# lixirui142/VidToMe

Hardware: AMD Instinct MI355X
Metric: denoising steps/sec, 16-frame 512x512 SD-1.5 chunk, ratio=0.5 (higher is better)
Workload: dtype f16 tokens; matching f16-MFMA filter + f32 exact refine (f32-identical indices); attention f16 MFMA with f32 accumulate

## Files before the change

vidtome_amd/csrc/match_filter.hip:

```cpp
#include "common.h"
#include "ablate.h"
#include "match_plan.h"

#include <algorithm>
#include <type_traits>

namespace {

using namespace vtm_match_plan;
static_assert(MODE_SCOUT_RANGE == VTM_MATCH_SCOUT_RANGE, "match_plan.h restates the public mode value");
constexpr int THREADS = 256;
constexpr float SCALE = 1024.0f;
constexpr float INV_S2 = 1.0f / (1024.0f * 1024.0f);
constexpr float WINDOW = SRC_LO ? 6.5e-4f : DST_LO ? 1.5e-3f : 2.4e-3f;
constexpr int MAX_C = 1280;

typedef float f32x16 __attribute__((ext_vector_type(16)));
typedef _Float16 h16x8 __attribute__((ext_vector_type(8)));
typedef uint32_t u32x4 __attribute__((ext_vector_type(4)));
typedef __attribute__((address_space(3))) void lds_void;
typedef const __attribute__((address_space(1))) void glb_void;

using vtm::to_f32;

template <typename T>
__device__ __forceinline__ const T *pool_row(const T *x0, int64_t P0, const T *x1, int64_t P1, int64_t b,
                                             int64_t r, int64_t C) {
    return r < P0 ? x0 + (b * P0 + r) * C : x1 + (b * P1 + (r - P0)) * C;
}

template <typename T>
__device__ __forceinline__ void load8(const T *src, float (&f)[8]) {
    if constexpr (sizeof(T) == 4) {
        const float4 v0 = *reinterpret_cast<const float4 *>(src);
        const float4 v1 = *reinterpret_cast<const float4 *>(src + 4);
        f[0] = v0.x; f[1] = v0.y; f[2] = v0.z; f[3] = v0.w;
        f[4] = v1.x; f[5] = v1.y; f[6] = v1.z; f[7] = v1.w;
    } else {
        const uint4 v = *reinterpret_cast<const uint4 *>(src);
        const T *e = reinterpret_cast<const T *>(&v);
#pragma unroll
        for (int j = 0; j < 8; ++j) f[j] = to_f32(e[j]);
    }
}

__device__ __forceinline__ float vmax3(float a, float b, float c) {
    float d;
    asm("v_max3_f32 %0, %1, %2, %3" : "=v"(d) : "v"(a), "v"(b), "v"(c));
    return d;
}
__device__ __forceinline__ float vmax2(float a, float b) {
    float d;
    asm("v_max_f32 %0, %1, %2" : "=v"(d) : "v"(a), "v"(b));
    return d;
}

struct RowDivisor {
    float n, r1, lo;
};
__device__ __forceinline__ RowDivisor row_divisor(float n) {
    const float r = __builtin_amdgcn_rcpf(n);
    const float e = __builtin_fmaf(-n, r, 1.0f);
    return {n, __builtin_fmaf(e, r, r), fmaxf(0x1p-102f, n * 0x1p-124f)};
}
__device__ __forceinline__ bool div_ok(float x, const RowDivisor &d) { return __builtin_fabsf(x) >= d.lo || x == 0.0f; }
__device__ __forceinline__ float div_by_row(float x, const RowDivisor &d) {
    const float q = x * d.r1;
    const float t = __builtin_fmaf(-d.n, q, x);
    const float q1 = __builtin_fmaf(t, d.r1, q);
    const float t2 = __builtin_fmaf(-d.n, q1, x);
    return __builtin_fmaf(t2, d.r1, q1);
}

__device__ __forceinline__ uint32_t orderable(float f) {
    if (f != f) return 0xffffffffu;
    const uint32_t u = __float_as_uint(f + 0.0f);
    return (u & 0x80000000u) ? ~u : (u | 0x80000000u);
}
__device__ __forceinline__ float from_orderable(uint32_t o) {
    if (o == 0u) return -INFINITY;
    return __uint_as_float((o & 0x80000000u) ? (o & 0x7fffffffu) : ~o);
}

struct SplitArgs {
    const int32_t *rows;
    int64_t n;
    float *norms;
    uint4 *out_hi, *out_lo;
    int64_t n_pad;
    float *rest, *tile_rest;
    float *rest2, *tile_rest2;
};

#ifndef VTM_PREP_PIECES
#define VTM_PREP_PIECES 10
#endif
constexpr int PREP_PIECES = VTM_PREP_PIECES;
constexpr int PREP_STRIDE = PREP_PIECES * 16 + 16;

template <typename T>
__global__ __launch_bounds__(64 * PREP_WAVES) void prep_operand(const T *__restrict__ x0, int64_t P0,
                                                    const T *__restrict__ x1, int64_t P1, int64_t B, int64_t C,
                                                    SplitArgs A0, SplitArgs A1, int64_t C_pad,
                                                    uint32_t *__restrict__ zero, int64_t zero_words,
                                                    unsigned long long *__restrict__ best, int64_t nbest, int64_t cut,
                                                    int64_t cut2) {
    static_assert(sizeof(T) == 2 || sizeof(T) == 4, "element size");
    static_assert(PREP_WAVES % 2 == 0, "a 128-row tile is two waves of one workgroup");
    __shared__ float wave_rest[PREP_WAVES], wave_rest2[PREP_WAVES];
    constexpr int EPP = 16 / (int)sizeof(T);
    __shared__ __attribute__((aligned(16))) char slab[PREP_WAVES][64 * PREP_STRIDE];
    const int64_t G = C_pad / 8;
    const int64_t gid = (int64_t)blockIdx.x * blockDim.x + threadIdx.x, gsz = (int64_t)gridDim.x * blockDim.x;
    for (int64_t w = gid; w < zero_words; w += gsz) zero[w] = 0u;
    for (int64_t w = gid; w < nbest; w += gsz) best[w] = 0ull;
    const int lane = threadIdx.x & 63, wave = threadIdx.x >> 6;
    char *my = slab[wave];

    int64_t idx = gid;
    const bool second = idx >= B * A0.n_pad;
    if (second) idx -= B * A0.n_pad;
    const SplitArgs &A = second ? A1 : A0;
    const int64_t n = A.n, n_pad = A.n_pad;
    const bool in_range = idx < B * n_pad;
    const int64_t i = in_range ? idx % n_pad : 0, b = in_range ? idx / n_pad : 0;
    const bool real = in_range && i < n;
    const T *src = real ? pool_row(x0, P0, x1, P1, b, A.rows[b * n + i], C) : x0;

    const int pieces = (int)(C * sizeof(T) / 16);
    const int nchunks = (pieces + PREP_PIECES - 1) / PREP_PIECES;
    uint4 stage[PREP_PIECES];
    auto issue = [&](int chunk) {
#pragma unroll
        for (int t = 0; t < PREP_PIECES; ++t) {
            const int q = lane + 64 * t, r = q / PREP_PIECES, col = q % PREP_PIECES;
            const T *rp = reinterpret_cast<const T *>(__shfl((unsigned long long)reinterpret_cast<uintptr_t>(src), r, 64));
            const int piece = chunk * PREP_PIECES + col;
            stage[t] = piece < pieces ? *reinterpret_cast<const uint4 *>(rp + (int64_t)piece * EPP) : make_uint4(0, 0, 0, 0);
        }
    };
    auto to_lds = [&]() {
#pragma unroll
        for (int t = 0; t < PREP_PIECES; ++t) {
            const int q = lane + 64 * t, r = q / PREP_PIECES, col = q % PREP_PIECES;
            *reinterpret_cast<uint4 *>(my + r * PREP_STRIDE + col * 16) = stage[t];
        }
    };
    auto my_piece = [&](int col, float (&f)[EPP]) {
        const uint4 v = *reinterpret_cast<const uint4 *>(my + lane * PREP_STRIDE + col * 16);
        const T *e = reinterpret_cast<const T *>(&v);
#pragma unroll
        for (int k = 0; k < EPP; ++k) f[k] = to_f32(e[k]);
    };

    float acc = 0.0f;
    issue(0);
    for (int c = 0; c < nchunks; ++c) {
        to_lds();
        if (c + 1 < nchunks) issue(c + 1);
        const int valid = min(PREP_PIECES, pieces - c * PREP_PIECES);
        for (int col = 0; col < valid; ++col) {
            float f[EPP];
            my_piece(col, f);
#pragma unroll
            for (int k = 0; k < EPP; ++k) acc = __builtin_fmaf(f[k], f[k], acc);
        }
    }
    const float nrm = __builtin_sqrtf(acc);
    if (real) A.norms[b * n + i] = nrm;

    const float rscale = SCALE * __builtin_amdgcn_rcpf(nrm);
    uint4 *__restrict__ out_hi = in_range ? A.out_hi + (b * G) * n_pad + i : nullptr;
    uint4 *__restrict__ out_lo = (in_range && A.out_lo) ? A.out_lo + (b * G) * n_pad + i : nullptr;
    constexpr int PPG = 8 / EPP;
    float rest = 0.0f, rest2 = 0.0f;
    issue(0);
    for (int c = 0; c < nchunks; ++c) {
        to_lds();
        if (c + 1 < nchunks) issue(c + 1);
        const int valid = min(PREP_PIECES, pieces - c * PREP_PIECES);
        for (int col = 0; col + PPG <= valid; col += PPG) {
            float f[8];
            if constexpr (PPG == 1) {
                my_piece(col, f);
            } else {
                float f0[EPP], f1[EPP];
                my_piece(col, f0);
                my_piece(col + 1, f1);
#pragma unroll
                for (int k = 0; k < EPP; ++k) { f[k] = f0[k]; f[EPP + k] = f1[k]; }
            }
            uint4 vh, vl;
            _Float16 *ph = reinterpret_cast<_Float16 *>(&vh), *pl = reinterpret_cast<_Float16 *>(&vl);
#pragma unroll
            for (int e = 0; e < 8; ++e) {
                const float sc = DST_LO ? (f[e] / nrm) * SCALE : f[e] * rscale;
                const _Float16 h = (_Float16)sc;
                ph[e] = h;
                pl[e] = (_Float16)(sc - (float)h);
            }
            if (!real) vh = vl = make_uint4(0, 0, 0, 0);
            const int64_t g = ((int64_t)c * PREP_PIECES + col) / PPG;
            if (g * 8 >= cut2) {
                float sq = 0.0f;
#pragma unroll
                for (int e = 0; e < 8; ++e) sq = __builtin_fmaf((float)ph[e], (float)ph[e], sq);
                rest2 += sq;
                if (g * 8 >= cut) rest += sq;
            }
            if (in_range) {
                out_hi[g * n_pad] = vh;
                if (out_lo) out_lo[g * n_pad] = vl;
            }
        }
    }
    if (in_range)
        for (int64_t g = C / 8; g < G; ++g) {
            out_hi[g * n_pad] = make_uint4(0, 0, 0, 0);
            if (out_lo) out_lo[g * n_pad] = make_uint4(0, 0, 0, 0);
        }
    const bool bad_row = real && !(nrm >= 0x1p-100f && nrm <= 0x1p100f);
    const float rnorm = !real ? 0.0f : bad_row ? INFINITY : __builtin_sqrtf(rest) * (1.0f + 0x1p-16f);
    if (in_range && A.rest) A.rest[b * n_pad + i] = rnorm;
    float wm = rnorm;
#pragma unroll
    for (int off = 32; off > 0; off >>= 1) wm = fmaxf(wm, __shfl_xor(wm, off, 64));
    if (lane == 0) wave_rest[wave] = wm;
    const float rnorm2 = !real ? 0.0f : bad_row ? INFINITY : __builtin_sqrtf(rest2) * (1.0f + 0x1p-16f);
    if (in_range && A.rest2) A.rest2[b * n_pad + i] = rnorm2;
    float wm2 = rnorm2;
#pragma unroll
    for (int off = 32; off > 0; off >>= 1) wm2 = fmaxf(wm2, __shfl_xor(wm2, off, 64));
    if (lane == 0) wave_rest2[wave] = wm2;
    __syncthreads();
    if (in_range && A.tile_rest && (threadIdx.x & 127) == 0)
        A.tile_rest[(b * n_pad + i) / 128] = fmaxf(wave_rest[wave], wave_rest[wave + 1]);
    if (in_range && A.tile_rest2 && (threadIdx.x & 127) == 0)
        A.tile_rest2[(b * n_pad + i) / 128] = fmaxf(wave_rest2[wave], wave_rest2[wave + 1]);
}

template <bool SCOUT>
__global__ __launch_bounds__(THREADS, 2) void filter_kernel(
    const uint4 *__restrict__ ah, const uint4 *__restrict__ al, const uint4 *__restrict__ bh,
    const uint4 *__restrict__ bl, int64_t Ns, int64_t Nd, int64_t Ns_pad, int64_t Nd_pad, int64_t C_pad, int align,
    int ns_tiles, int nd_tiles, int nsplit, int tiles_per_split, int total_src_tiles, int patch_tiles,
    unsigned int *__restrict__ amax, int *__restrict__ cnt, uint2 *__restrict__ cand, int cand_rows, int *__restrict__ flags,
    const float *__restrict__ rest_a, const float *__restrict__ rest_bt, int KP, int count_blocks,
    unsigned int *__restrict__ tilemap, int map_words) {
    __shared__ __attribute__((aligned(16))) uint4 sA[2][DST_LO ? 2 : 1][8 * FBD];

    const int tid = threadIdx.x, lane = tid & 63;
    const int wave = __builtin_amdgcn_readfirstlane(tid >> 6);
    const int l31 = lane & 31, kh = lane >> 5;

    const int xcd = blockIdx.x & 7, slot = blockIdx.x >> 3;
    const int per_group = patch_tiles * nsplit;
    const int grp = (slot / per_group) * 8 + xcd;
    const int q = slot % per_group;
    const int stg = grp * patch_tiles + q % patch_tiles;
    const int split = q / patch_tiles;
    if (stg >= total_src_tiles) return;
    const int st_ = stg % ns_tiles;
    const int bi = stg / ns_tiles;
    int jt0 = split * tiles_per_split;
    int jt1 = min(jt0 + tiles_per_split, nd_tiles);
    if (jt0 >= jt1) return;
    if constexpr (!SCOUT) {
        if (tilemap != nullptr) {
            const unsigned int *row = tilemap + (int64_t)stg * map_words;
            int lo = jt1, hi = jt0;
            for (int w = jt0 >> 5; w <= (jt1 - 1) >> 5; ++w) {
                unsigned int bits = row[w];
                if (w == (jt0 >> 5)) bits &= 0xffffffffu << (jt0 & 31);
                if (w == ((jt1 - 1) >> 5) && (jt1 & 31)) bits &= 0xffffffffu >> (32 - (jt1 & 31));
                if (bits) {
                    lo = min(lo, w * 32 + __ffs(bits) - 1);
                    hi = max(hi, w * 32 + 32 - __clz(bits));
                }
            }
            lo = __builtin_amdgcn_readfirstlane(lo);
            hi = __builtin_amdgcn_readfirstlane(hi);
            if (lo >= hi) return;
            jt0 = lo;
            jt1 = hi;
        }
    }

    const int KT = SCOUT ? KP : (int)(C_pad / FBK);
    const int64_t G = C_pad / 8;
    const int steps = (jt1 - jt0) * KT;
    int n_tested = 0, n_alive = 0;
    const uint4 *srch = ah + (int64_t)bi * G * Ns_pad, *srcl = al + (int64_t)bi * G * Ns_pad;
    const uint4 *dsth = bh + (int64_t)bi * G * Nd_pad, *dstl = bl + (int64_t)bi * G * Nd_pad;
    const int64_t srow0 = (int64_t)st_ * FBS + wave * 64;

    constexpr int NB = SRC_LO ? 4 : 2;
    const uint32_t voff_b = (uint32_t)(kh * Ns_pad + srow0 + l31) * 16u;
    const int64_t bgroup = 2 * Ns_pad;
    u32x4 rb[4][2][2];
    [[maybe_unused]] auto load_b = [&](int kt, int ks, u32x4 (&dst)[2][2]) {
        const uint4 *ph = srch + (int64_t)ABL_STREAMED(kt * 4 + ks, ks) * bgroup;
        asm volatile("global_load_dwordx4 %0, %1, %2" : "=v"(dst[0][0]) : "v"(voff_b), "s"(ph));
        asm volatile("global_load_dwordx4 %0, %1, %2 offset:512" : "=v"(dst[1][0]) : "v"(voff_b), "s"(ph));
        if constexpr (SRC_LO) {
            const uint4 *pl = srcl + (int64_t)(kt * 4 + ks) * bgroup;
            asm volatile("global_load_dwordx4 %0, %1, %2" : "=v"(dst[0][1]) : "v"(voff_b), "s"(pl));
            asm volatile("global_load_dwordx4 %0, %1, %2 offset:512" : "=v"(dst[1][1]) : "v"(voff_b), "s"(pl));
        }
    };
    auto await_b = [&](auto count_tag, u32x4 (&r)[2][2]) {
        constexpr int N = decltype(count_tag)::value;
        if constexpr (SRC_LO)
            asm volatile("s_waitcnt vmcnt(%4)" : "+v"(r[0][0]), "+v"(r[1][0]), "+v"(r[0][1]), "+v"(r[1][1]) : "n"(N));
        else
            asm volatile("s_waitcnt vmcnt(%2)" : "+v"(r[0][0]), "+v"(r[1][0]) : "n"(N));
    };
    constexpr int NPIECE = DST_LO ? 8 : 4, PG = NPIECE / 2;
    const uint4 *abase[NPIECE];
    uint32_t alds[NPIECE];
#pragma unroll
    for (int t = 0; t < NPIECE; ++t) {
        const int q = wave * NPIECE + t, which = q >> 4, qq = q & 15, p = qq >> 1, half = qq & 1;
        abase[t] = (which ? dstl : dsth) + (int64_t)p * Nd_pad + half * 64;
        alds[t] = (uint32_t)reinterpret_cast<uintptr_t>((lds_void *)&sA[0][which][p * FBD + half * 64]);
    }
    const uint32_t voff_a = (uint32_t)lane * 16u;
    [[maybe_unused]] auto load_a_half = [&](int jt, int kt, int buf, int half_id) {
        const int64_t step_off = ABL_STREAMED((int64_t)kt * 8 * Nd_pad + (int64_t)jt * FBD, (int64_t)0);
#pragma unroll
        for (int t = 0; t < PG; ++t) {
            const uint4 *g = abase[half_id * PG + t] + step_off;
            const uint32_t lds_off = alds[half_id * PG + t] + (uint32_t)buf * (uint32_t)sizeof(sA[0]);
            asm volatile("s_mov_b32 m0, %0\n\ts_nop 0\n\tglobal_load_lds_dwordx4 %1, %2"
                         :
                         : "s"(lds_off), "v"(voff_a), "s"(g)
                         : "memory");
        }
    };

    f32x16 acc[4][2];

    const int64_t out_row0 = align ? 0 : (int64_t)bi * Ns;
    const uint32_t idx_base = align ? (uint32_t)((int64_t)bi * Nd) : 0u;
    constexpr float WS = WINDOW * SCALE * SCALE;
    float runmax[2], cv[2][4];
    uint32_t ci[2][4];
    float rest_l[2];
    uint32_t live = 0xffu;
    auto push = [&](int64_t srow, float v_scaled, uint32_t d) -> bool {
        const int slot = atomicAdd(&cnt[out_row0 + srow], 1);
        if (slot < CAP)
            cand[(uint32_t)slot * (uint32_t)cand_rows + (uint32_t)(out_row0 + srow)] = make_uint2(__float_as_uint(v_scaled * INV_S2), d + idx_base);
        return slot >= CAP;
    };
#pragma unroll
    for (int sb = 0; sb < 2; ++sb) {
        const int64_t srow = srow0 + sb * 32 + l31;
        runmax[sb] = srow < Ns ? from_orderable(amax[out_row0 + srow]) * (SCALE * SCALE)
                               : INFINITY;
        rest_l[sb] = rest_a ? rest_a[(int64_t)bi * Ns_pad + srow] : 0.0f;
#pragma unroll
        for (int e = 0; e < 4; ++e) {
            cv[sb][e] = -INFINITY;
            ci[sb][e] = 0;
        }
    }

    uint32_t am[2] = {0u, 0u};
// ... 670 lines not shown
#pragma unroll
            for (int g = 0; g < 4; ++g) {
                float4 af[4];
#pragma unroll
                for (int ib = 0; ib < 4; ++ib) af[ib] = *reinterpret_cast<const float4 *>(&sD[((g * 2 + kh) * XPD + ib * 32 + l31) * 4]);
                float bv[XSB][4];
#pragma unroll
                for (int sb = 0; sb < XSB; ++sb) {
                    const float4 bf = *reinterpret_cast<const float4 *>(&sS[((g * 2 + kh) * XPS + wave * (32 * XSB) + sb * 32 + l31) * 4]);
                    bv[sb][0] = bf.x; bv[sb][1] = bf.y; bv[sb][2] = bf.z; bv[sb][3] = bf.w;
                }
#pragma unroll
                for (int e = 0; e < 4; ++e) {
#pragma unroll
                    for (int ib = 0; ib < 4; ++ib) {
                        const float av = e == 0 ? af[ib].x : e == 1 ? af[ib].y : e == 2 ? af[ib].z : af[ib].w;
#pragma unroll
                        for (int sb = 0; sb < XSB; ++sb) {
                            f32x16 c = acc[ib][sb];
                            if (kt == 0 && g == 0 && e == 0) {
#pragma unroll
                                for (int r = 0; r < 16; ++r) c[r] = 0.0f;
                            }
                            acc[ib][sb] = __builtin_amdgcn_mfma_f32_32x32x2f32(av, bv[sb][e], c, 0, 0, 0);
                        }
                    }
                }
            }
            if (wrap) {
                const int dst0 = jt * XD + 4 * kh;
                const bool full = (int64_t)(jt + 1) * XD <= Nd;
#pragma unroll
                for (int sb = 0; sb < XSB; ++sb) {
                    float bv_ = bestv[sb];
                    uint32_t bi_ = besti[sb];
#pragma unroll
                    for (int ib = 0; ib < 4; ++ib) {
#pragma unroll
                        for (int r = 0; r < 16; ++r) {
                            const int d = dst0 + ib * 32 + (r & 3) + 8 * (r >> 2);
                            const float sc = acc[ib][sb][r];
                            bool upd = !(sc <= bv_) && (bv_ == bv_);
                            uint32_t od = (uint32_t)d;
                            if constexpr (ORD) {
                                od = sOrd[jt & 1][d - jt * XD];
                                upd = upd || (((sc == bv_) || (sc != sc && bv_ != bv_)) && od < bi_);
                            }
                            if (!full) upd = upd && (d < Nd);
                            bv_ = upd ? sc : bv_;
                            bi_ = upd ? od : bi_;
                        }
                    }
                    bestv[sb] = bv_;
                    besti[sb] = bi_;
                }
                ++jt;
                kt = 0;
            } else if (can_prune && kt + 1 == KX) {
                const float rb = rest_bt[bi * rest_tiles + jt] * (1.0f + 0x1p-9f) * INV_S2;
                bool dead = true;
#pragma unroll
                for (int sb = 0; sb < XSB; ++sb) {
                    float pm = -INFINITY;
#pragma unroll
                    for (int ib = 0; ib < 4; ++ib)
#pragma unroll
                        for (int r = 0; r < 16; ++r) pm = fmaxf(pm, acc[ib][sb][r]);
                    dead = dead && (pm + rest_l[sb] * rb + 1e-4f < fmaxf(bestv[sb], floor_[sb]));
                }
                if (__syncthreads_and(dead)) {
                    ++jt;
                    kt = 0;
                    if (jt < jt1) {
                        dst_rows(jt);
                        fetch(0);
                    }
                } else {
                    ++kt;
                }
            } else {
                ++kt;
            }
        }
#pragma unroll
        for (int sb = 0; sb < XSB; ++sb) {
            const int64_t i = listed(wave * (32 * XSB) + sb * 32 + l31);
            if (i >= 0 && besti[sb] != 0xffffffffu) {
                const uint32_t col = besti[sb] + (align ? (uint32_t)(bi * Nd) : 0u);
                const int64_t orow = align ? (ORD ? (int64_t)src_order[i] : i) : l * Ns + (ORD ? (int64_t)src_order[l * Ns + i] : i);
                atomicMax(&best[orow], ((unsigned long long)orderable(bestv[sb]) << 32) | (uint32_t)(~col));
            }
        }
        item = next_item();
    }
}

struct Workspace {
    float *na, *nb;
    uint4 *ah, *al, *bh, *bl;
    unsigned int *amax, *seedlb, *tilemap;
    int *cnt, *flags, *ovf_rows, *ovf_cnt;
    uint2 *cand, *pairs;
    float *rest_a, *rest_bt, *rest_a2, *rest_bt2;
    int64_t zero_words;

    Workspace(void *ws, const Layout &L) : zero_words((int64_t)((L.cand - L.amax) / 4)) {
        auto at = [ws](auto *&p, size_t off) { p = reinterpret_cast<std::remove_reference_t<decltype(p)>>(static_cast<char *>(ws) + off); };
        at(na, L.na), at(nb, L.nb), at(ah, L.ah), at(al, L.al), at(bh, L.bh), at(bl, L.bl), at(amax, L.amax), at(seedlb, L.seedlb);
        at(tilemap, L.tilemap), at(cnt, L.cnt), at(flags, L.flags), at(ovf_rows, L.ovf), at(ovf_cnt, L.ovf_cnt), at(cand, L.cand);
        at(pairs, L.pairs), at(rest_a, L.rest_a), at(rest_bt, L.rest_bt), at(rest_a2, L.rest_a2), at(rest_bt2, L.rest_bt2);
    }
};

int32_t *kernel_writable(int32_t *flags_out) {
    if (!flags_out) return nullptr;
    hipPointerAttribute_t attr;
    if (hipPointerGetAttributes(&attr, flags_out) == hipSuccess &&
        (attr.type == hipMemoryTypeDevice || attr.type == hipMemoryTypeHost || attr.type == hipMemoryTypeManaged))
        return attr.type == hipMemoryTypeHost && attr.devicePointer ? (int32_t *)attr.devicePointer : flags_out;
    (void)hipGetLastError();
    return nullptr;
}
}

VTM_EXPORT size_t vtm_match_filtered_ws_bytes(int64_t B, int64_t C, int64_t Ns, int64_t Nd, int align) {
    if (B <= 0 || C <= 0 || Ns <= 0 || Nd <= 0) return 0;
    return make_layout(B, C, Ns, Nd, align).total;
}

static int match_filtered_impl(const void *x0, int64_t P0, const void *x1, int64_t P1, int dtype, int64_t B,
                               int64_t C, const int32_t *a_rows, int64_t Ns, const int32_t *b_rows, int64_t Nd,
                               int align, void *ws, size_t ws_bytes, uint64_t *best, int32_t *flags_out,
                               int64_t seed_L, int64_t seed_N, const int32_t *seed_pos1, const int32_t *seed_table,
                               int mode, const int32_t *src_order, const int32_t *dst_order, vtm_stream_t stream) {
    const char *what = "vtm_match_filtered";
    VTM_REQUIRE(x0 && a_rows && b_rows && ws && best, "vtm_match_filtered: null pointer");
    const int scout_steps = (mode >> 8) & 0xff;
    mode &= 0xff;
    VTM_REQUIRE((src_order == nullptr) == (dst_order == nullptr), "vtm_match_filtered_ordered: both inverse maps or none");
    VTM_REQUIRE(mode == VTM_MATCH_ONE_LAUNCH || mode == VTM_MATCH_SCOUT_RANGE, "vtm_match_filtered: bad mode %d", mode);
    VTM_REQUIRE(B > 0 && C > 0 && C % 8 == 0 && Ns > 0 && Nd > 0, "vtm_match_filtered: bad sizes");
    VTM_REQUIRE(P1 == 0 || x1, "vtm_match_filtered: x1 is null but P1 > 0");
    VTM_REQUIRE(B * Nd < (1ll << 32) - 1, "vtm_match_filtered: index space overflow");
    VTM_REQUIRE(C <= MAX_C, "vtm_match_filtered: C=%lld > %d (error window derived for C <= %d; use vtm_match)",
                (long long)C, MAX_C, MAX_C);
    const Layout L = make_layout(B, C, Ns, Nd, align);
    if (ws_bytes < L.total)
        return vtm::fail(VTM_EWORKSPACE, "vtm_match_filtered: workspace %zu < %zu bytes", ws_bytes, L.total);
    const int64_t rows_out = align ? Ns : B * Ns;
    VTM_REQUIRE(rows_out * CAP < (1ll << 31), "vtm_match_filtered: too many rows for the 32-bit candidate index");
    VTM_REQUIRE(dtype == VTM_F32 || dtype == VTM_F16 || dtype == VTM_BF16, "vtm_match_filtered: bad dtype");

    const DebugEnv &dbg = debug_env();
    const FilterPlan P = plan_filter(L, B, C, Ns, Nd, align, mode, scout_steps, seed_N, src_order != nullptr, vtm::device_cus(), dbg);
    const Workspace W(ws, L);
    hipStream_t s = vtm::as_stream(stream);
    unsigned long long *bp = reinterpret_cast<unsigned long long *>(best);
    const dim3 block(256);
    const bool shallow = P.KPS < P.KP;

    vtm::with_dtype(dtype, what, [&](auto t) {
        using T = decltype(t);
        const SplitArgs A0{a_rows, Ns, W.na, W.ah, SRC_LO ? W.al : nullptr, L.Ns_pad, W.rest_a, nullptr, shallow ? W.rest_a2 : nullptr, nullptr};
        const SplitArgs A1{b_rows, Nd, W.nb, W.bh, DST_LO ? W.bl : nullptr, L.Nd_pad, nullptr, W.rest_bt, nullptr, shallow ? W.rest_bt2 : nullptr};
        hipLaunchKernelGGL(prep_operand<T>, dim3(P.prep_grid), dim3(64 * PREP_WAVES), 0, s, (const T *)x0, P0, (const T *)x1, P1,
                           B, C, A0, A1, L.C64, W.amax, W.zero_words, bp, rows_out, P.cut, P.cut2);
        return VTM_OK;
    });
    if (P.seed_grid)
        vtm::with_dtype(dtype, what, [&](auto t) {
            using T = decltype(t);
            const int dry = dbg.seed_dry;
            const float lb_margin = (4.0f * (float)C + 32.0f) * 0x1p-24f + 1e-6f;
            hipLaunchKernelGGL(seed_kernel<T>, dim3(P.seed_grid), block, 0, s, (const T *)x0, P0, (const T *)x1, P1, B, C, a_rows,
                               Ns, b_rows, Nd, (const float *)W.na, (const float *)W.nb, align, seed_L, seed_N, seed_pos1, seed_table,
                               W.amax, dry, W.seedlb, lb_margin);
            return VTM_OK;
        });

    auto filter = [&](auto kernel, int64_t grid, int nsplit, int tps, const float *rest_a, const float *rest_bt, int kp,
                      unsigned int *tilemap) {
        hipLaunchKernelGGL(kernel, dim3((unsigned)grid), dim3(THREADS), 0, s, W.ah, W.al, W.bh, W.bl, Ns, Nd, L.Ns_pad, L.Nd_pad,
                           L.C64, align, P.ns_tiles, P.nd_tiles, nsplit, tps, P.total_src_tiles, P.patch_tiles, W.amax, W.cnt, W.cand,
                           (int)rows_out, W.flags, rest_a, rest_bt, kp, flags_out != nullptr ? 1 : 0, tilemap, P.map_words);
    };
    if (P.range_plan) {
        filter(filter_kernel<true>, P.grid, P.nsplit, P.tiles_per_split, shallow ? W.rest_a2 : W.rest_a,
               shallow ? W.rest_bt2 : W.rest_bt, P.KPS, W.tilemap);
        filter(filter_kernel<false>, P.grid_r, P.nsplit_r, P.tps_r, W.rest_a, W.rest_bt, P.KP, W.tilemap);
    } else {
        filter(filter_kernel<false>, P.grid, P.nsplit, P.tiles_per_split, P.prune ? W.rest_a : nullptr,
               P.prune ? W.rest_bt : nullptr, P.prune ? P.KP : 0x7fffffff, nullptr);
    }

    int32_t *flags_pub = kernel_writable(flags_out);
    vtm::with_dtype(dtype, what, [&](auto t) {
        using T = decltype(t);
        hipLaunchKernelGGL(refine_kernel<T>, dim3(P.refine_grid), block, 0, s, (const T *)x0, P0, (const T *)x1, P1, B, C, a_rows, Ns,
                           b_rows, Nd, W.na, W.nb, align, W.flags, rows_out, W.amax, W.cnt, W.cand, W.ovf_cnt, W.ovf_rows, W.pairs,
                           (const float *)W.rest_bt, B * (L.Nd_pad / FBD), bp, src_order, dst_order);
        hipLaunchKernelGGL((src_order ? exact_rows_kernel<T, true> : exact_rows_kernel<T, false>), dim3(P.xgrid), block, 0, s,
                           (const T *)x0, P0, (const T *)x1, P1, B, C, a_rows, Ns, b_rows, Nd, W.na, W.nb, align, W.flags, W.ovf_cnt,
                           W.ovf_rows, bp, P.xsplit, P.xtps, (const float *)W.rest_a, (const float *)W.rest_bt, P.KX, L.Ns_pad,
                           L.Nd_pad / FBD, (const unsigned int *)W.seedlb, W.flags + 6, src_order, dst_order, flags_pub);
        return VTM_OK;
    });
    if (int rc = vtm::launch_status(what)) return rc;

    if (flags_out && !flags_pub) {
        const hipError_t e = hipMemcpyAsync(flags_out, W.flags, 8 * sizeof(int), hipMemcpyDefault, s);
        if (e != hipSuccess) return vtm::fail(VTM_ELAUNCH, "vtm_match_filtered: copy: %s", hipGetErrorString(e));
    }
    return VTM_OK;
}

VTM_EXPORT int vtm_match_filtered(const void *x0, int64_t P0, const void *x1, int64_t P1, int dtype, int64_t B,
                                  int64_t C, const int32_t *a_rows, int64_t Ns, const int32_t *b_rows, int64_t Nd,
                                  int align, void *ws, size_t ws_bytes, uint64_t *best, int32_t *flags_out,
                                  vtm_stream_t stream) {
    return match_filtered_impl(x0, P0, x1, P1, dtype, B, C, a_rows, Ns, b_rows, Nd, align, ws, ws_bytes, best, flags_out, 0, 0,
                               nullptr, nullptr, VTM_MATCH_ONE_LAUNCH, nullptr, nullptr, stream);
}

VTM_EXPORT int vtm_match_filtered_seeded(const void *x0, int64_t P0, const void *x1, int64_t P1, int dtype, int64_t B,
                                         int64_t C, const int32_t *a_rows, int64_t Ns, const int32_t *b_rows, int64_t Nd,
                                         int align, void *ws, size_t ws_bytes, uint64_t *best, int32_t *flags_out,
                                         int64_t seed_L, int64_t seed_N, const int32_t *seed_pos1, const int32_t *seed_table,
                                         vtm_stream_t stream) {
    VTM_REQUIRE(seed_N >= 0 && seed_L >= 0, "vtm_match_filtered_seeded: bad seed description");
    return match_filtered_impl(x0, P0, x1, P1, dtype, B, C, a_rows, Ns, b_rows, Nd, align, ws, ws_bytes, best, flags_out, seed_L,
                               seed_N, seed_pos1, seed_table, VTM_MATCH_ONE_LAUNCH, nullptr, nullptr, stream);
}

VTM_EXPORT int vtm_match_filtered_plan(const void *x0, int64_t P0, const void *x1, int64_t P1, int dtype, int64_t B,
                                       int64_t C, const int32_t *a_rows, int64_t Ns, const int32_t *b_rows, int64_t Nd,
                                       int align, void *ws, size_t ws_bytes, uint64_t *best, int32_t *flags_out,
                                       int64_t seed_L, int64_t seed_N, const int32_t *seed_pos1, const int32_t *seed_table,
                                       int mode, vtm_stream_t stream) {
    VTM_REQUIRE(seed_N >= 0 && seed_L >= 0, "vtm_match_filtered_plan: bad seed description");
    return match_filtered_impl(x0, P0, x1, P1, dtype, B, C, a_rows, Ns, b_rows, Nd, align, ws, ws_bytes, best, flags_out, seed_L,
                               seed_N, seed_pos1, seed_table, mode, nullptr, nullptr, stream);
}

VTM_EXPORT int vtm_match_filtered_ordered(const void *x0, int64_t P0, const void *x1, int64_t P1, int dtype, int64_t B,
                                          int64_t C, const int32_t *a_sorted, int64_t Ns, const int32_t *b_sorted, int64_t Nd,
                                          int align, void *ws, size_t ws_bytes, uint64_t *best, int32_t *flags_out, int64_t seed_L,
                                          int64_t seed_N, const int32_t *seed_pos1, const int32_t *seed_table, int mode,
                                          const int32_t *a_order, const int32_t *b_order, vtm_stream_t stream) {
    VTM_REQUIRE(seed_N >= 0 && seed_L >= 0, "vtm_match_filtered_ordered: bad seed description");
    VTM_REQUIRE(a_order && b_order, "vtm_match_filtered_ordered: null inverse map");
    return match_filtered_impl(x0, P0, x1, P1, dtype, B, C, a_sorted, Ns, b_sorted, Nd, align, ws, ws_bytes, best, flags_out, seed_L,
                               seed_N, seed_pos1, seed_table, mode, a_order, b_order, stream);
}

namespace vtm {
int filter_ablations() { return VTM_ABLATIONS; }
}
```

vidtome_amd/csrc/match_plan.h:

```cpp
#pragma once
#include <cstddef>
#include <cstdint>
#include <cstdlib>

namespace vtm_match_plan {

constexpr int FBD = 128;
constexpr int FBS = 256;
constexpr int FBK = 64;
constexpr int CAP = 64;
#ifndef VTM_FILTER_PRODUCTS
#define VTM_FILTER_PRODUCTS 1
#endif
constexpr bool SRC_LO = VTM_FILTER_PRODUCTS >= 3;
constexpr bool DST_LO = VTM_FILTER_PRODUCTS >= 2;
static_assert(DST_LO || !SRC_LO, "the src lo half is only used together with the dst lo half");
#ifndef VTM_PREP_WAVES
#define VTM_PREP_WAVES 4
#endif
constexpr int PREP_WAVES = VTM_PREP_WAVES;
#ifndef VTM_RROWS
#define VTM_RROWS 64
#endif
constexpr int RROWS = VTM_RROWS;
#ifndef VTM_XS
#define VTM_XS 128
#endif
constexpr int XS = VTM_XS;
constexpr int XD = 128;
constexpr int XK = 32;
constexpr int MODE_SCOUT_RANGE = 1;

inline int64_t cdiv(int64_t a, int64_t b) { return (a + b - 1) / b; }
inline size_t align_up(size_t v) { return (v + 255) & ~(size_t)255; }

struct Layout {
    size_t na, nb, ah, al, bh, bl, amax, cnt, seedlb, tilemap, cand, flags, ovf_cnt, ovf, pairs, rest_a, rest_bt, rest_a2, rest_bt2, total;
    int64_t Ns_pad, Nd_pad, C64;
};

inline Layout make_layout(int64_t B, int64_t C, int64_t Ns, int64_t Nd, int align) {
    Layout L;
    L.Ns_pad = cdiv(Ns, FBS) * FBS;
    L.Nd_pad = cdiv(Nd, FBS) * FBS;
    L.C64 = cdiv(C, 64) * 64;
    const int64_t rows_out = align ? Ns : B * Ns;
    size_t o = 0;
    auto take = [&](size_t bytes) { size_t at = o; o += align_up(bytes); return at; };
    L.na = take((size_t)B * Ns * 4);
    L.nb = take((size_t)B * Nd * 4);
    L.ah = take((size_t)B * L.C64 * L.Ns_pad * 2);
    L.al = take(SRC_LO ? (size_t)B * L.C64 * L.Ns_pad * 2 : 0);
    L.bh = take((size_t)B * L.C64 * L.Nd_pad * 2);
    L.bl = take(DST_LO ? (size_t)B * L.C64 * L.Nd_pad * 2 : 0);
    L.amax = take((size_t)rows_out * 4);
    L.cnt = take((size_t)rows_out * 4);
    L.seedlb = take((size_t)rows_out * 4);
    L.tilemap = take((size_t)B * (L.Ns_pad / FBS) * ((L.Nd_pad / FBD + 31) / 32) * 4);
    L.flags = take(256);
    L.ovf_cnt = take((size_t)B * 4);
    L.cand = take((size_t)rows_out * CAP * 8);
    L.ovf = take((size_t)rows_out * 4);
    L.pairs = take((size_t)rows_out * CAP * 8);
    L.rest_a = take((size_t)B * L.Ns_pad * 4);
    L.rest_bt = take((size_t)B * (L.Nd_pad / FBD) * 4);
    L.rest_a2 = take((size_t)B * L.Ns_pad * 4);
    L.rest_bt2 = take((size_t)B * (L.Nd_pad / FBD) * 4);
    L.total = o;
    return L;
}

struct DebugEnv {
    int kp5, kp, nsplit;
    bool seed_dry, nsplit_r4, no_xprune;
};
inline const DebugEnv &debug_env() {
    static const DebugEnv e = [] {
        auto num = [](const char *name) {
            const char *v = getenv(name);
            return v ? atoi(v) : -1;
        };
        DebugEnv d;
        d.kp5 = num("VTM_DEBUG_KP5");
        d.kp = num("VTM_DEBUG_KP");
        d.nsplit = num("VTM_DEBUG_NSPLIT");
        d.seed_dry = getenv("VTM_DEBUG_SEED_DRY") != nullptr;
        d.nsplit_r4 = getenv("VTM_DEBUG_NSPLIT_R4") != nullptr;
        d.no_xprune = getenv("VTM_DEBUG_NOXPRUNE") != nullptr;
        return d;
    }();
    return e;
}

struct FilterPlan {
    int KT, KP, KPS;
    bool prune;
    int64_t cut, cut2;
    int ns_tiles, nd_tiles, total_src_tiles, patch_tiles, ngroups;
    int nsplit, tiles_per_split;
    int64_t grid;
    bool range_plan;
    int tps_r, nsplit_r;
    int64_t grid_r;
    int map_words;
    int xsplit, xtps, KX;
    unsigned xgrid, refine_grid, prep_grid, seed_grid;
};

inline int wgs_per_xcd(int nd_tiles, int patch_wgs, int ns) {
    const int tps = (int)cdiv(nd_tiles, ns);
    return patch_wgs * (int)cdiv(nd_tiles, tps);
}

inline int nsplit_rounds_1_4(int nd_tiles, int patch_wgs, int ns_tiles, int64_t B, int cus) {
    int64_t want = cdiv(1536, (int64_t)ns_tiles * B);
    int nsplit = (int)(want < 1 ? 1 : want);
    if (nd_tiles >= 32) nsplit = 8;
    if (nsplit > nd_tiles / 4) nsplit = nd_tiles / 4 > 0 ? nd_tiles / 4 : 1;
    if (nsplit > 8) nsplit = 8;
    if (nsplit == 8) {
        const int slots = cus / 8 * 2;
        for (int ns = 7; ns >= 6; --ns)
            if (wgs_per_xcd(nd_tiles, patch_wgs, 8) > slots && wgs_per_xcd(nd_tiles, patch_wgs, ns) <= slots) return ns;
    }
    return nsplit;
}

inline int nsplit_round_5(int nd_tiles, int patch_wgs, int cus) {
    const int slots = cus / 8 * 2;
    double best_cost = 1e30;
    int nsplit = 1;
    for (int ns = 1; ns <= 16 && ns <= nd_tiles; ++ns) {
        const int tps = (int)cdiv(nd_tiles, ns);
        if ((int)cdiv(nd_tiles, tps) != ns) continue;
        if (tps < 4 && ns > 1) continue;
        const int wgs = wgs_per_xcd(nd_tiles, patch_wgs, ns);
        const double rounds = (wgs <= slots && wgs > slots - slots / 16) ? 2.0 : (double)cdiv(wgs, slots);
        const double cost = rounds * (tps + 1.5) + 0.25 * ns;
        if (cost < best_cost - 1e-9) {
            best_cost = cost;
            nsplit = ns;
        }
    }
    return nsplit;
}

inline FilterPlan plan_filter(const Layout &L, int64_t B, int64_t , int64_t Ns, int64_t Nd, int align, int mode,
                              int scout_steps, int64_t seed_N, bool ordered, int cus, const DebugEnv &dbg) {
    FilterPlan P;
    const int KT = P.KT = (int)(L.C64 / FBK);
    int KP = (VTM_FILTER_PRODUCTS == 1 && KT >= 4) ? (2 * KT + 2) / 5 : 0;
    if (VTM_FILTER_PRODUCTS == 1 && KT == 5 && dbg.kp5 >= 0 && dbg.kp5 < KT) KP = dbg.kp5;
    if (VTM_FILTER_PRODUCTS == 1 && dbg.kp >= 0 && dbg.kp < KT) KP = dbg.kp;
    P.KP = KP;
    P.prune = KP > 0 && KP < KT;
    P.cut = P.prune ? (int64_t)KP * FBK : L.C64;
    P.KPS = (P.prune && mode == MODE_SCOUT_RANGE && scout_steps > 0 && scout_steps < KP) ? scout_steps : KP;
    P.cut2 = P.KPS < KP ? (int64_t)P.KPS * FBK : P.cut;

    const int ns_tiles = P.ns_tiles = (int)(L.Ns_pad / FBS), nd_tiles = P.nd_tiles = (int)(L.Nd_pad / FBD);
    P.total_src_tiles = (int)(B * ns_tiles);
    const int max_patch = (int64_t)16 * FBS * L.C64 * 2 <= (3 << 20) ? 16 : 8;
    const int tiles_per_xcd = (int)cdiv(P.total_src_tiles, 8);
    const int patches_per_xcd = (int)cdiv(tiles_per_xcd, max_patch);
    P.patch_tiles = (int)cdiv(tiles_per_xcd, patches_per_xcd);
    P.ngroups = (int)cdiv(P.total_src_tiles, P.patch_tiles);
    const int patch_wgs = patches_per_xcd * P.patch_tiles;
    int nsplit = dbg.nsplit_r4 ? nsplit_rounds_1_4(nd_tiles, patch_wgs, ns_tiles, B, cus) : nsplit_round_5(nd_tiles, patch_wgs, cus);
    if (dbg.nsplit >= 1 && dbg.nsplit <= 16 && dbg.nsplit <= nd_tiles) nsplit = dbg.nsplit;
    P.tiles_per_split = (int)cdiv(nd_tiles, nsplit);
    P.nsplit = (int)cdiv(nd_tiles, P.tiles_per_split);
    P.grid = (int64_t)8 * cdiv(P.ngroups, 8) * P.patch_tiles * P.nsplit;
    P.map_words = (nd_tiles + 31) / 32;
    P.range_plan = mode == MODE_SCOUT_RANGE && P.prune &&
                   (ordered ? seed_N > 0 && nd_tiles >= 2 : seed_N >= 2 * FBD && seed_N % FBD == 0);
    P.tps_r = !P.range_plan ? 0 : ordered ? P.tiles_per_split : (int)(seed_N / FBD);
    P.nsplit_r = P.range_plan ? (int)cdiv(nd_tiles, P.tps_r) : 0;
    P.grid_r = (int64_t)8 * cdiv(P.ngroups, 8) * P.patch_tiles * P.nsplit_r;

    const int xd_tiles = (int)cdiv(Nd, XD);
    int xsplit = xd_tiles / 8;
    xsplit = xsplit < 1 ? 1 : xsplit > 16 ? 16 : xsplit;
    P.xtps = (int)cdiv(xd_tiles, xsplit);
    P.xsplit = (int)cdiv(xd_tiles, P.xtps);
    P.xgrid = (unsigned)((XS == 128 ? 2 : 1) * cus);
    P.KX = dbg.no_xprune ? 0 : (int)(P.cut / XK);

    P.refine_grid = (unsigned)cdiv(align ? Ns : B * Ns, RROWS);
    P.prep_grid = (unsigned)cdiv(B * (L.Ns_pad + L.Nd_pad), 64 * PREP_WAVES);
    P.seed_grid = seed_N > 0 ? (unsigned)cdiv(B * Ns * 8, 256) : 0u;
    return P;
}

}
```

Baseline: 22.06.

## Add single-pass register-resident prep kernel for 16-bit tokens with LDS transpose

Adds a prep_single_pass kernel for f16/bf16 tokens with C up to 640. Each wave loads its 64 rows into registers with coalesced 16-byte pieces, using shuffled row pointers and an LDS slab to transpose them. The norm and the scaled hi/lo split are then computed from registers instead of re-reading global memory in a second pass. The aim is to halve global reads and improve coalescing in the prep stage, at the cost of higher register pressure and LDS use; the chunked path stays selectable through an env var.

```diff
diff --git a/vidtome_amd/csrc/match_filter.hip b/vidtome_amd/csrc/match_filter.hip
--- a/vidtome_amd/csrc/match_filter.hip
+++ b/vidtome_amd/csrc/match_filter.hip
@@ -20,6 +20,7 @@
 typedef uint32_t u32x4 __attribute__((ext_vector_type(4)));
 typedef __attribute__((address_space(3))) void lds_void;
 typedef const __attribute__((address_space(1))) void glb_void;
+typedef __attribute__((address_space(1))) u32x4 glb_u32x4;
 
 using vtm::to_f32;
 
@@ -214,6 +215,143 @@
             }
         }
     }
+    if (in_range)
+        for (int64_t g = C / 8; g < G; ++g) {
+            out_hi[g * n_pad] = make_uint4(0, 0, 0, 0);
+            if (out_lo) out_lo[g * n_pad] = make_uint4(0, 0, 0, 0);
+        }
+    const bool bad_row = real && !(nrm >= 0x1p-100f && nrm <= 0x1p100f);
+    const float rnorm = !real ? 0.0f : bad_row ? INFINITY : __builtin_sqrtf(rest) * (1.0f + 0x1p-16f);
+    if (in_range && A.rest) A.rest[b * n_pad + i] = rnorm;
+    float wm = rnorm;
+#pragma unroll
+    for (int off = 32; off > 0; off >>= 1) wm = fmaxf(wm, __shfl_xor(wm, off, 64));
+    if (lane == 0) wave_rest[wave] = wm;
+    const float rnorm2 = !real ? 0.0f : bad_row ? INFINITY : __builtin_sqrtf(rest2) * (1.0f + 0x1p-16f);
+    if (in_range && A.rest2) A.rest2[b * n_pad + i] = rnorm2;
+    float wm2 = rnorm2;
+#pragma unroll
+    for (int off = 32; off > 0; off >>= 1) wm2 = fmaxf(wm2, __shfl_xor(wm2, off, 64));
+    if (lane == 0) wave_rest2[wave] = wm2;
+    __syncthreads();
+    if (in_range && A.tile_rest && (threadIdx.x & 127) == 0)
+        A.tile_rest[(b * n_pad + i) / 128] = fmaxf(wave_rest[wave], wave_rest[wave + 1]);
+    if (in_range && A.tile_rest2 && (threadIdx.x & 127) == 0)
+        A.tile_rest2[(b * n_pad + i) / 128] = fmaxf(wave_rest2[wave], wave_rest2[wave + 1]);
+}
+
+constexpr int RES_PIECES = 10;
+constexpr int RES_STRIDE = RES_PIECES * 16 + 16;
+static_assert(RES_PIECES * 8 * 4 == PREP_SINGLE_CHANNELS, "match_plan.h restates the channels of four blocks");
+
+template <typename T, int BLOCKS>
+__global__ __launch_bounds__(64 * PREP_WAVES, BLOCKS <= 4 ? 2 : 1) void prep_single_pass(
+    const T *__restrict__ x0, int64_t P0, const T *__restrict__ x1, int64_t P1, int64_t B, int64_t C, SplitArgs A0, SplitArgs A1,
+    int64_t C_pad, uint32_t *__restrict__ zero, int64_t zero_words, unsigned long long *__restrict__ best, int64_t nbest,
+    int64_t cut, int64_t cut2) {
+    static_assert(sizeof(T) == 2, "16-bit tokens: a 16-byte piece is one 8-channel panel group");
+    constexpr int ROW = BLOCKS * RES_PIECES;
+    __shared__ float wave_rest[PREP_WAVES], wave_rest2[PREP_WAVES];
+    __shared__ __attribute__((aligned(16))) char slab[PREP_WAVES][64 * RES_STRIDE];
+    const int64_t G = C_pad / 8;
+    const int64_t gid = (int64_t)blockIdx.x * blockDim.x + threadIdx.x, gsz = (int64_t)gridDim.x * blockDim.x;
+    for (int64_t w = gid; w < zero_words; w += gsz) zero[w] = 0u;
+    for (int64_t w = gid; w < nbest; w += gsz) best[w] = 0ull;
+    const int lane = threadIdx.x & 63, wave = threadIdx.x >> 6;
+    char *my = slab[wave];
+
+    int64_t idx = gid;
+    const bool second = idx >= B * A0.n_pad;
+    if (second) idx -= B * A0.n_pad;
+    const SplitArgs &A = second ? A1 : A0;
+    const int64_t n = A.n, n_pad = A.n_pad;
+    const bool in_range = idx < B * n_pad;
+    const int64_t i = in_range ? idx % n_pad : 0, b = in_range ? idx / n_pad : 0;
+    const bool real = in_range && i < n;
+    const T *src = real ? pool_row(x0, P0, x1, P1, b, A.rows[b * n + i], C) : x0;
+
+    const int pieces = (int)(C / 8);
+    u32x4 own[ROW];
+    const glb_u32x4 *p[RES_PIECES];
+#pragma unroll
+    for (int t = 0; t < RES_PIECES; ++t) {
+        const int q = lane + 64 * t;
+        p[t] = reinterpret_cast<const glb_u32x4 *>(
+                   __shfl((unsigned long long)reinterpret_cast<uintptr_t>(src), q / RES_PIECES, 64)) + q % RES_PIECES;
+    }
+    if (pieces == ROW) {
+#pragma unroll
+        for (int t = 0; t < RES_PIECES; ++t)
+#pragma unroll
+            for (int blk = 0; blk < BLOCKS; ++blk) own[blk * RES_PIECES + t] = p[t][blk * RES_PIECES];
+    } else {
+#pragma unroll
+        for (int t = 0; t < RES_PIECES; ++t)
+#pragma unroll
+            for (int blk = 0; blk < BLOCKS; ++blk)
+                own[blk * RES_PIECES + t] =
+                    (lane + 64 * t) % RES_PIECES + blk * RES_PIECES < pieces ? p[t][blk * RES_PIECES] : u32x4{0u, 0u, 0u, 0u};
+    }
+#pragma unroll
+    for (int blk = 0; blk < BLOCKS; ++blk) {
+#pragma unroll
+        for (int t = 0; t < RES_PIECES; ++t) {
+            const int q = lane + 64 * t;
+            *reinterpret_cast<u32x4 *>(my + (q / RES_PIECES) * RES_STRIDE + (q % RES_PIECES) * 16) = own[blk * RES_PIECES + t];
+        }
+#pragma unroll
+        for (int col = 0; col < RES_PIECES; ++col)
+            own[blk * RES_PIECES + col] = *reinterpret_cast<const u32x4 *>(my + lane * RES_STRIDE + col * 16);
+    }
+
+    float acc = 0.0f;
+#pragma unroll
+    for (int col = 0; col < ROW; ++col)
+        if (col < pieces) {
+            const T *e = reinterpret_cast<const T *>(&own[col]);
+#pragma unroll
+            for (int k = 0; k < 8; ++k) {
+                const float f = to_f32(e[k]);
+                acc = __builtin_fmaf(f, f, acc);
+            }
+        }
+    const float nrm = __builtin_sqrtf(acc);
+    if (real) A.norms[b * n + i] = nrm;
+
+    const float rscale = SCALE * __builtin_amdgcn_rcpf(nrm);
+    uint4 *__restrict__ out_hi = in_range ? A.out_hi + (b * G) * n_pad + i : nullptr;
+    uint4 *__restrict__ out_lo = (in_range && A.out_lo) ? A.out_lo + (b * G) * n_pad + i : nullptr;
+    float rest = 0.0f, rest2 = 0.0f;
+#pragma unroll
+    for (int g = 0; g < ROW; ++g)
+        if (g < pieces) {
+            asm("" : "+v"(own[g]));
+            const T *x = reinterpret_cast<const T *>(&own[g]);
+            uint4 vh, vl;
+            _Float16 *ph = reinterpret_cast<_Float16 *>(&vh), *pl = reinterpret_cast<_Float16 *>(&vl);
+#pragma unroll
+            for (int e = 0; e < 8; ++e) {
+                const float f = to_f32(x[e]);
+                float sc = DST_LO ? (f / nrm) * SCALE : f * rscale;
+                asm("" : "+v"(sc));
+                const _Float16 h = (_Float16)sc;
+                ph[e] = h;
+                if constexpr (DST_LO) pl[e] = (_Float16)(sc - (float)h);
+            }
+            if (!real) vh = vl = make_uint4(0, 0, 0, 0);
+            if (g * 8 >= cut2) {
+                float sq = 0.0f;
+#pragma unroll
+                for (int e = 0; e < 8; ++e) sq = __builtin_fmaf((float)ph[e], (float)ph[e], sq);
+                rest2 += sq;
+                if (g * 8 >= cut) rest += sq;
+            }
+            if (in_range) {
+                out_hi[g * n_pad] = vh;
+                if constexpr (DST_LO)
+                    if (out_lo) out_lo[g * n_pad] = vl;
+            }
+        }
     if (in_range)
         for (int64_t g = C / 8; g < G; ++g) {
             out_hi[g * n_pad] = make_uint4(0, 0, 0, 0);
@@ -1190,7 +1328,8 @@
     VTM_REQUIRE(dtype == VTM_F32 || dtype == VTM_F16 || dtype == VTM_BF16, "vtm_match_filtered: bad dtype");
 
     const DebugEnv &dbg = debug_env();
-    const FilterPlan P = plan_filter(L, B, C, Ns, Nd, align, mode, scout_steps, seed_N, src_order != nullptr, vtm::device_cus(), dbg);
+    const FilterPlan P = plan_filter(L, B, C, Ns, Nd, align, mode, scout_steps, seed_N, src_order != nullptr, vtm::device_cus(), dbg,
+                                     dtype == VTM_F32 ? 4 : 2);
     const Workspace W(ws, L);
     hipStream_t s = vtm::as_stream(stream);
     unsigned long long *bp = reinterpret_cast<unsigned long long *>(best);
@@ -1201,8 +1340,15 @@
         using T = decltype(t);
         const SplitArgs A0{a_rows, Ns, W.na, W.ah, SRC_LO ? W.al : nullptr, L.Ns_pad, W.rest_a, nullptr, shallow ? W.rest_a2 : nullptr, nullptr};
         const SplitArgs A1{b_rows, Nd, W.nb, W.bh, DST_LO ? W.bl : nullptr, L.Nd_pad, nullptr, W.rest_bt, nullptr, shallow ? W.rest_bt2 : nullptr};
-        hipLaunchKernelGGL(prep_operand<T>, dim3(P.prep_grid), dim3(64 * PREP_WAVES), 0, s, (const T *)x0, P0, (const T *)x1, P1,
-                           B, C, A0, A1, L.C64, W.amax, W.zero_words, bp, rows_out, P.cut, P.cut2);
+        auto prep = [&](auto kernel, unsigned grid) {
+            hipLaunchKernelGGL(kernel, dim3(grid), dim3(64 * PREP_WAVES), 0, s, (const T *)x0, P0, (const T *)x1, P1, B, C, A0, A1,
+                               L.C64, W.amax, W.zero_words, bp, rows_out, P.cut, P.cut2);
+        };
+        if constexpr (sizeof(T) == 2) {
+            if (P.prep_blocks == 4) prep(prep_single_pass<T, 4>, P.prep_single_grid);
+            if (P.prep_blocks == 8) prep(prep_single_pass<T, 8>, P.prep_single_grid);
+        }
+        if (P.prep_blocks == 0) prep(prep_operand<T>, P.prep_grid);
         return VTM_OK;
     });
     if (P.seed_grid)
diff --git a/vidtome_amd/csrc/match_plan.h b/vidtome_amd/csrc/match_plan.h
--- a/vidtome_amd/csrc/match_plan.h
+++ b/vidtome_amd/csrc/match_plan.h
@@ -2,6 +2,7 @@
 #include <cstddef>
 #include <cstdint>
 #include <cstdlib>
+#include <cstring>
 
 namespace vtm_match_plan {
 
@@ -19,6 +20,7 @@
 #define VTM_PREP_WAVES 4
 #endif
 constexpr int PREP_WAVES = VTM_PREP_WAVES;
+constexpr int PREP_SINGLE_CHANNELS = 320;
 #ifndef VTM_RROWS
 #define VTM_RROWS 64
 #endif
@@ -73,6 +75,7 @@
 struct DebugEnv {
     int kp5, kp, nsplit;
     bool seed_dry, nsplit_r4, no_xprune;
+    bool prep_chunked;
 };
 inline const DebugEnv &debug_env() {
     static const DebugEnv e = [] {
@@ -87,6 +90,8 @@
         d.seed_dry = getenv("VTM_DEBUG_SEED_DRY") != nullptr;
         d.nsplit_r4 = getenv("VTM_DEBUG_NSPLIT_R4") != nullptr;
         d.no_xprune = getenv("VTM_DEBUG_NOXPRUNE") != nullptr;
+        const char *prep = getenv("VTM_DEBUG_PREP");
+        d.prep_chunked = prep != nullptr && std::strcmp(prep, "chunked") == 0;
         return d;
     }();
     return e;
@@ -105,6 +110,8 @@
     int map_words;
     int xsplit, xtps, KX;
     unsigned xgrid, refine_grid, prep_grid, seed_grid;
+    int prep_blocks;
+    unsigned prep_single_grid;
 };
 
 inline int wgs_per_xcd(int nd_tiles, int patch_wgs, int ns) {
@@ -145,8 +152,8 @@
     return nsplit;
 }
 
-inline FilterPlan plan_filter(const Layout &L, int64_t B, int64_t , int64_t Ns, int64_t Nd, int align, int mode,
-                              int scout_steps, int64_t seed_N, bool ordered, int cus, const DebugEnv &dbg) {
+inline FilterPlan plan_filter(const Layout &L, int64_t B, int64_t C, int64_t Ns, int64_t Nd, int align, int mode,
+                              int scout_steps, int64_t seed_N, bool ordered, int cus, const DebugEnv &dbg, int elem_bytes = 2) {
     FilterPlan P;
     const int KT = P.KT = (int)(L.C64 / FBK);
     int KP = (VTM_FILTER_PRODUCTS == 1 && KT >= 4) ? (2 * KT + 2) / 5 : 0;
@@ -189,6 +196,8 @@
     P.refine_grid = (unsigned)cdiv(align ? Ns : B * Ns, RROWS);
     P.prep_grid = (unsigned)cdiv(B * (L.Ns_pad + L.Nd_pad), 64 * PREP_WAVES);
     P.seed_grid = seed_N > 0 ? (unsigned)cdiv(B * Ns * 8, 256) : 0u;
+    P.prep_blocks = (dbg.prep_chunked || elem_bytes != 2 || C > 2 * PREP_SINGLE_CHANNELS) ? 0 : C > PREP_SINGLE_CHANNELS ? 8 : 4;
+    P.prep_single_grid = P.prep_blocks ? (unsigned)cdiv(B * (L.Ns_pad + L.Nd_pad), 64 * PREP_WAVES) : 0u;
     return P;
 }
 
```

Result: no change. 22.22, median of 6 (+0.7%).
